# fuine/katome

Measured on AMD Instinct MI355X. Metric: k-mers/s, higher is better.
Workload: dtype u64

## Files before the change

### katome_amd/csrc/common.h

```cpp
#pragma once
#include <hip/hip_runtime.h>
#include <errno.h>
#include <stdarg.h>
#include <stdint.h>
#include <stdio.h>
#include <string.h>
#include <chrono>
#include <type_traits>
#include <vector>

#include "../../include/katome_gpu.h"
#include "env.h"
#include "kmer_bits.h"

namespace katome {

void set_error(const char* fmt, ...);
const char* get_error();

#define KCHECK_HIP(expr)                                                                         \
    do {                                                                                         \
        hipError_t _e = (expr);                                                                  \
        if (_e != hipSuccess) {                                                                  \
            katome::set_error("HIP error %d (%s) at %s:%d: %s", (int)_e, hipGetErrorString(_e),  \
// ... 144 lines not shown
    if (k < 3 || k > 63) { set_error("k = %u unsupported (3..63)", k); return KATOME_E_UNSUPPORTED; }
    return KATOME_OK;
}

constexpr int BLOCK = 256;
#ifdef __HIPCC__
__device__ __forceinline__ u32 wave_sum(u32 v) {
#pragma unroll
    for (int o = 32; o > 0; o >>= 1) v += __shfl_down(v, o, 64);
    return v;
}
#endif
inline unsigned grid_for(uint64_t work_items, unsigned per_block, unsigned cap = 256u * 16u) {
    uint64_t g = (work_items + per_block - 1) / per_block;
    if (g < 1) g = 1;
    return (unsigned)(g > cap ? cap : g);
}
#define KLAUNCH(kernel, n, stream, ...) hipLaunchKernelGGL(kernel, dim3(grid_for((n), BLOCK, 256u * 32u)), dim3(BLOCK), 0, stream, __VA_ARGS__)
inline double now_ms() { return std::chrono::duration<double, std::milli>(std::chrono::steady_clock::now().time_since_epoch()).count(); }

template <bool B> using BoolC = std::integral_constant<bool, B>;
template <int I> using IntC = std::integral_constant<int, I>;
template <class F> int with_bool(bool b, F f) { return b ? f(BoolC<true>{}) : f(BoolC<false>{}); }

int launch_extract_fixed(uint32_t k, bool rc, const uint8_t* d_packed, uint64_t n_reads, uint32_t read_len,
                         const uint8_t* d_skip, uint64_t* d_records, hipStream_t stream, uint32_t span = 1, bool mark = false,
                         uint32_t first_window = 0, uint32_t records_per_read = 0);
bool extract_tile_counts_ok(uint32_t k, uint32_t read_len, uint32_t span, uint32_t sort_tile, const uint8_t* d_packed, const uint64_t* d_records);
int launch_extract_tiles_counted(uint32_t k, bool rc, const uint8_t* d_packed, uint64_t n_reads, uint32_t read_len, uint32_t span,
                                 uint64_t* d_records, uint32_t* d_counts, uint32_t sort_tile, hipStream_t stream);
int launch_extract_var(uint32_t k, bool rc, const uint8_t* d_packed, uint64_t packed_bytes, const uint64_t* d_byte_off,
                       const uint32_t* d_len, const uint64_t* d_win_prefix, uint64_t n_reads, uint64_t total_windows,
                       uint64_t* d_records, hipStream_t stream, bool mark = false, uint32_t span = 1, uint32_t mode = 0);

int dev_sort(uint64_t* d_keys, uint32_t* d_vals, uint64_t n, uint32_t nw, uint32_t key_bits, hipStream_t stream);
struct DevBuf;
int dev_sort_bufs(DevBuf& keys, DevBuf* vals, uint64_t n, uint32_t nw, uint32_t key_bits, hipStream_t stream, bool distinct_keys = false);
int dev_partition(const uint64_t* d_in, const uint32_t* v_in, uint64_t n, uint32_t nw, uint32_t n_parts, uint64_t* d_out,
                  uint32_t* v_out, uint64_t* h_counts, hipStream_t stream, uint32_t core_shift = 0, uint32_t core_bases = 0, uint32_t minimizer = 0);
constexpr uint32_t SUPERMER_M = 11;
uint32_t supermer_slots(uint32_t k, uint32_t read_len, uint32_t m);
bool supermer_route_takes(uint32_t k, uint32_t read_len, uint32_t m);
int dev_supermers_extract(const uint8_t* d_packed, uint64_t n_reads, uint32_t read_len, const uint8_t* d_skip, uint32_t k, uint32_t m, bool rc,
                          uint32_t n_owners, uint32_t slots, uint64_t* d_out, uint64_t* d_spill, uint64_t spill_cap, uint64_t* d_spill_cursor,
                          hipStream_t stream);
int dev_supermers_expand(const uint64_t* d_list, const uint32_t* d_counts, uint64_t n, uint32_t k, bool rc, DevBuf& keys, DevBuf& weights,
                         uint64_t* n_records, hipStream_t stream);
int dev_partition_supermers(const uint64_t* d_in, uint64_t n, uint32_t n_parts, uint64_t* d_out, uint64_t* h_counts, hipStream_t stream);
int dev_partition_range(const uint64_t* d_vals, const uint32_t* idx_in, uint64_t n, const uint64_t* d_bounds, uint32_t n_parts,
                        uint64_t* d_out, uint32_t* idx_out, uint64_t* h_counts, hipStream_t stream);
int dev_hash_order_core(const uint64_t* d_in, const uint32_t* w_in, uint64_t n, uint32_t core_shift, uint32_t core_bases, uint64_t* ka, uint64_t* kb,
                        uint32_t* wa, uint32_t* wb, const uint64_t** k_out, const uint32_t** w_out, uint32_t* group_bits, hipStream_t stream);
inline bool fused_records_on() { static const bool on = env_flag("KATOME_FUSED_RECORDS", true); return on; }
struct RecordSource {
    const uint64_t* tiles = nullptr; const uint32_t* counts = nullptr;
    uint64_t n_tiles = 0;
    uint32_t tile_bases = 0, k = 0, span = 0, stride = 0;
    bool rc = false, rep = false, pending = false;
    DevBuf* keys = nullptr; DevBuf* weights = nullptr;
    size_t key_bytes = 0, weight_bytes = 0;
    hipStream_t stream = nullptr;
    DevBuf own_tiles, own_counts;
    uint64_t n_records() const { return n_tiles * span; }
    int first_pass_done() {
        pending = false; tiles = nullptr; counts = nullptr;
        own_tiles.release(); own_counts.release();
        if (int rc = keys->alloc(key_bytes, stream)) return rc;
        return weights->alloc(weight_bytes, stream);
    }
};
bool fused_records_takes(uint32_t nwt, uint32_t nwk, bool rep, uint32_t span);
int table_materialise_records(RecordSource& src);
int dev_hash_order_tagged(const uint64_t* d_in, const uint32_t* w_in, uint64_t n, uint32_t nwk, uint64_t* ka, uint64_t* kb, uint32_t* wa, uint32_t* wb,
                          const uint64_t** k_out, const uint32_t** w_out, uint32_t* group_bits, hipStream_t stream, uint32_t* first_counts = nullptr);
int dev_region_order(const uint64_t* d_in, const uint32_t* w_in, uint64_t n, uint32_t nw, int passes, uint64_t* ka, uint64_t* kb,
                     uint32_t* wa, uint32_t* wb, const uint64_t** k_out, const uint32_t** w_out, hipStream_t stream);
int dev_hash_order(const uint64_t* d_in, const uint32_t* w_in, uint64_t n, uint32_t nw, uint64_t* ka, uint64_t* kb, uint32_t* wa, uint32_t* wb,
                   const uint64_t** k_out, const uint32_t** w_out, uint32_t* group_bits, hipStream_t stream, uint32_t* first_counts = nullptr,
                   RecordSource* src = nullptr);
uint32_t dev_sort_tile_keys(uint32_t nw);
inline bool fused_hist_on() { static const bool on = env_flag("KATOME_FUSED_HIST", true); return on; }
int dev_key_order(const uint64_t* d_in, const uint32_t* w_in, uint64_t n, uint32_t k, uint64_t* ka, uint64_t* kb, uint32_t* wa, uint32_t* wb,
                  const uint64_t** k_out, const uint32_t** w_out, hipStream_t stream, uint32_t* first_counts = nullptr,
                  const uint8_t* first_digits = nullptr, RecordSource* src = nullptr);
int dev_list_first_pass(const uint64_t* d_tiles, const uint32_t* d_counts, uint64_t n_tiles, uint32_t tile_bases, uint32_t k, uint32_t span, uint32_t stride,
                        bool rc, bool rep, bool fused, uint64_t* d_keys, uint32_t* d_weights, uint32_t* d_digit_counts, hipStream_t stream);
int dev_s2_region_pass(const uint64_t* d_keys, const uint32_t* d_w, const uint8_t* d_digits, uint32_t k, const uint64_t* start, const uint64_t* used,
                       uint64_t* k_out, uint32_t* w_out, uint64_t* n_tiles, hipStream_t stream);
size_t dev_digit_stream_bytes(uint64_t n, uint32_t nw);
bool dev_digit_stream_pays(uint32_t nw);
int dev_key_group_index(const uint64_t* d_keys, uint64_t n, uint32_t shift, uint64_t* d_index, hipStream_t stream);
int dev_half_merge(const uint64_t* a_key, const uint32_t* a_w, const uint64_t* a_first, const uint32_t* a_count, const uint64_t* a_off,
                   const uint64_t* b_key, const uint32_t* b_w, const uint64_t* b_first, uint64_t* out_key, uint32_t* out_w, uint64_t n_out,
                   hipStream_t stream);
uint32_t dev_group_merge_cap();
uint64_t dev_source_head_blocks(uint64_t n_edges);
int dev_group_merge(const uint64_t* a_key, const uint32_t* a_w, const uint64_t* a_first, const uint32_t* a_count, const uint64_t* a_off,
                    const uint64_t* b_key, const uint32_t* b_w, const uint64_t* b_first, uint32_t k, uint64_t* out_key, uint32_t* out_w,
                    uint64_t n_out, hipStream_t stream, uint32_t* head_counts = nullptr);
int dev_key_group_max(const uint64_t* d_index, uint64_t* d_out, hipStream_t stream);
int dev_unique(uint64_t* d_keys, uint64_t n, uint32_t nw, uint64_t* n_out, hipStream_t stream);
int dev_rank(const uint64_t* d_sorted, uint64_t n_sorted, uint32_t nw, uint32_t key_bits, const uint64_t* d_q, uint64_t nq,
             uint64_t* d_out, hipStream_t stream);
int dev_bucket_index(const uint64_t* d_sorted, uint64_t n, uint32_t nw, uint32_t key_bits, uint32_t B, uint64_t* d_index, hipStream_t stream);
int dev_iota(uint32_t* d, uint64_t n, hipStream_t stream);
int dev_fill_u32(uint32_t* d, uint64_t n, uint32_t v, hipStream_t stream);
// ... 305 lines not shown
```

### katome_amd/csrc/radix.hip

```cpp
#include <algorithm>
#include <type_traits>

#include "common.h"
#include "edge_keys.h"
#include "lds_order.h"
#include "s2_regions.h"

namespace katome {

constexpr int RADIX_BITS = 8;
constexpr int RADIX = 1 << RADIX_BITS;
#ifndef KATOME_SORT_ITEMS
#define KATOME_SORT_ITEMS 16
#endif
#ifndef KATOME_SORT_ITEMS_WIDE
#define KATOME_SORT_ITEMS_WIDE 8
#endif
#ifndef KATOME_SORT_ITEMS_3
#define KATOME_SORT_ITEMS_3 5
#endif
#ifndef KATOME_SORT_WAVES
#define KATOME_SORT_WAVES 4
#endif
template <int NW> struct SortTile {
    static constexpr int ITEMS = NW == 1 ? KATOME_SORT_ITEMS : NW == 2 ? KATOME_SORT_ITEMS_WIDE : KATOME_SORT_ITEMS_3;
    static constexpr int KEYS = BLOCK * ITEMS;
};
static inline unsigned chunk_blocks_for(unsigned long long nblocks) {
    unsigned c = 64;
    while (c < 1024 && (unsigned long long)c * c < nblocks) c <<= 1;
    return c;
}
static_assert(BLOCK == RADIX, "one thread per digit in the offset kernels");

template <int NW> struct RadixDigit {
    u32 shift, bits;
    __device__ __forceinline__ u32 operator()(const Key<NW>& k) const { return key_digit(k, shift, bits); }
};
template <int NW> struct OwnerDigit {
    u64 n_parts;
    u32 core_shift, core_bases;
    u32 minimizer = 0;
    __device__ __forceinline__ u32 operator()(const Key<NW>& k0) const {
        if (!key_valid(k0)) return (u32)n_parts;
        Key<NW> k = k0;
        k.w[0] &= ~RC_MARK;
        if (minimizer) return (u32)minimizer_owner(k, core_shift, core_bases, minimizer, n_parts);
        return core_bases ? (u32)core_owner(k, core_shift, core_bases, n_parts) : (u32)whole_key_owner(k, n_parts);
    }
};
struct SupermerOwnerDigit {
    u32 n_parts;
    __device__ __forceinline__ u32 operator()(const Key<2>& k) const { return key_valid(k) ? supermer_owner(k) : n_parts; }
};
struct RangeDigit {
    const u64* bounds; u32 n_parts;
    __device__ __forceinline__ u32 operator()(const Key<1>& k) const {
// ... 112 lines not shown
    const u64 tile = nw == 1 ? SortTile<1>::KEYS : nw == 2 ? SortTile<2>::KEYS : SortTile<3>::KEYS;
    return (size_t)((n + tile - 1) / tile * tile);
}

__global__ __launch_bounds__(BLOCK) void radix_chunk_kernel(u32* __restrict__ counts, u64 nblocks, u64* __restrict__ chunk_sum, u32 chunk_blocks) {
    const u32 d = threadIdx.x;
    const u64 b0 = (u64)blockIdx.x * chunk_blocks;
    const u64 b1 = b0 + chunk_blocks < nblocks ? b0 + chunk_blocks : nblocks;
    u32 run = 0;
    constexpr int U = 8;
    u64 b = b0;
    for (; b + U <= b1; b += U) {
        u32 c[U];
#pragma unroll
        for (int j = 0; j < U; ++j) c[j] = counts[(b + j) * RADIX + d];
#pragma unroll
        for (int j = 0; j < U; ++j) { counts[(b + j) * RADIX + d] = run; run += c[j]; }
    }
    for (; b < b1; ++b) {
        u32 c = counts[b * RADIX + d];
        counts[b * RADIX + d] = run;
        run += c;
    }
    chunk_sum[(u64)blockIdx.x * RADIX + d] = run;
}

__global__ __launch_bounds__(BLOCK) void radix_offsets_kernel(u64* __restrict__ chunk_sum, u64 nchunks, u64* __restrict__ digit_total) {
    __shared__ u64 tot[RADIX];
    const u32 d = threadIdx.x;
    u64 t = 0;
    for (u64 c = 0; c < nchunks; ++c) t += chunk_sum[c * RADIX + d];
    tot[d] = t;
    if (digit_total) digit_total[d] = t;
    __syncthreads();
    u64 start = 0;
    for (u32 e = 0; e < d; ++e) start += tot[e];
    constexpr int U = 8;
    u64 c = 0;
    for (; c + U <= nchunks; c += U) {
        u64 v[U];
#pragma unroll
        for (int j = 0; j < U; ++j) v[j] = chunk_sum[(c + j) * RADIX + d];
#pragma unroll
        for (int j = 0; j < U; ++j) { chunk_sum[(c + j) * RADIX + d] = start; start += v[j]; }
    }
    for (; c < nchunks; ++c) {
        u64 v = chunk_sum[c * RADIX + d];
        chunk_sum[c * RADIX + d] = start;
        start += v;
    }
}

struct NoNextDigit {};
template <int NWT, int NWK, bool RC, bool REP> struct ListSource {
    static constexpr bool PLACED = false;
    const u64* tiles; const u32* counts; u32 k, span, stride, inv;
    struct Origin { u64 t0; u32 o0; };
    __device__ __forceinline__ Origin origin(u64 base) const { const u64 t0 = base / span; return Origin{t0, (u32)(base - t0 * span)}; }
    __device__ __forceinline__ void load(const Origin& at, u32 idx, Key<NWK>& key, u32& val) const {
        const u32 q = at.o0 + idx, tr = __umulhi(q, inv), o = q - tr * span;
        const u64 t = at.t0 + tr;
        Key<NWT> tile;
#pragma unroll
        for (int w = 0; w < NWT; ++w) tile.w[w] = tiles[t * NWT + w];
        key = level_orientation<NWK, RC, REP>(sub_window<NWT, NWK>(tile, k, span, stride, o), k);
        val = counts[t];
    }
};
template <class Next> struct NextDigitOut {
    Next nx; uint8_t* out;
    __device__ __forceinline__ void put(u64 at, u32 d) const { out[at] = (uint8_t)d; }
};
template <> struct NextDigitOut<NoNextDigit> {};
template <int NW, bool HAS_VAL, class Digit, bool STABLE = true, class Next = NoNextDigit, class Src = ArraySource>
__global__ __launch_bounds__(BLOCK, KATOME_SORT_WAVES) void radix_scatter_kernel(const u64* __restrict__ keys_in, const u32* __restrict__ vals_in,
                                                               u64 n, Digit dg, const u32* __restrict__ rel,
                                                               const u64* __restrict__ chunk_off, u64* __restrict__ keys_out,
                                                               u32* __restrict__ vals_out, u32 chunk_blocks, u32 xcd_tiles, NextDigitOut<Next> next, Src src) {
    constexpr bool NEXT = !std::is_same<Next, NoNextDigit>::value, PLACED = Src::PLACED, LISTED = !std::is_same<Src, ArraySource>::value && !PLACED;
    static_assert(!LISTED || HAS_VAL, "a list's records carry its counts");
    constexpr int SORT_ITEMS = SortTile<NW>::ITEMS, SORT_TILE = SortTile<NW>::KEYS;
    extern __shared__ u64 smem[];
    u64* skeys = smem;
    __shared__ u32 whist[BLOCK / 64][RADIX];
    __shared__ u32 dstart[RADIX];
    __shared__ u64 gbase[RADIX];
    __shared__ u32 wsum[BLOCK / 64];

    const u32 tid = threadIdx.x, lane = tid & 63, wave = tid >> 6;
    const u64 bid = xcd_tiles ? (u64)(blockIdx.x & 7u) * xcd_tiles + (blockIdx.x >> 3) : (u64)blockIdx.x;
    const u64 base = bid * SORT_TILE;
    if (base >= n) return;
    u32 cnt = (u32)((n - base) < (u64)SORT_TILE ? (n - base) : (u64)SORT_TILE);
    for (u32 i = tid; i < (BLOCK / 64) * RADIX; i += BLOCK) (&whist[0][0])[i] = 0;
    __syncthreads();

    Key<NW> key[SORT_ITEMS]; u32 val[SORT_ITEMS]; u32 dig[SORT_ITEMS]; u32 rnk[SORT_ITEMS];
    const u64 lt_mask = lane ? (~0ull >> (64 - lane)) : 0ull;
    const typename Src::Origin from = src.origin(base);
    u64 in0 = base;
    if constexpr (PLACED) { in0 = from.base; cnt = from.cnt; }
#pragma unroll
    for (int j = 0; j < SORT_ITEMS; ++j) {
        const u32 idx = wave * (64 * SORT_ITEMS) + j * 64 + lane;
        const bool valid = idx < cnt;
        u32 d = 0;
        if (valid) {
            if constexpr (LISTED) src.load(from, idx, key[j], val[j]);
            else {
#if KATOME_STREAM_LOADS >= 1
            key[j] = load_key_stream<NW>(keys_in, in0 + idx);
            if (HAS_VAL) val[j] = __builtin_nontemporal_load(&vals_in[in0 + idx]);
#else
            key[j] = load_key<NW>(keys_in, in0 + idx);
            if (HAS_VAL) val[j] = vals_in[in0 + idx];
#endif
            }
            d = dg(key[j]);
        }
        if (!STABLE) {
            dig[j] = d;
            rnk[j] = valid ? atomicAdd(&whist[0][d], 1u) : 0u;
            continue;
        }
        const u64 vmask = __ballot(valid);
        u32 diff_lo = 0, diff_hi = 0;
#pragma unroll
        for (int b = 0; b < RADIX_BITS; ++b) {
            const u32 mine = (u32)((int)(d << (31 - b)) >> 31);
            const u64 vote = __ballot(mine != 0);
            diff_lo |= (u32)vote ^ mine;
            diff_hi |= (u32)(vote >> 32) ^ mine;
        }
        const u64 m = ~((u64)diff_hi << 32 | diff_lo) & vmask;
        const u32 prior = __popcll(m & lt_mask);
        u32 old = 0;
        if (valid) old = whist[wave][d];
        if (valid && prior == 0) whist[wave][d] = old + __popcll(m);
        dig[j] = d;
        rnk[j] = old + prior;
    }
    __syncthreads();

    {
        const u32 d = tid;
        u32 run = 0;
        if (!STABLE) { run = whist[0][d]; whist[0][d] = 0; }
        else {
#pragma unroll
        for (int w = 0; w < BLOCK / 64; ++w) { u32 c = whist[w][d]; whist[w][d] = run; run += c; }
        }
        u32 incl = run;
#pragma unroll
        for (int o = 1; o < 64; o <<= 1) { u32 v = __shfl_up(incl, o, 64); if (lane >= (u32)o) incl += v; }
        if (lane == 63) wsum[wave] = incl;
        __syncthreads();
        u32 woff = 0;
#pragma unroll
        for (int w = 0; w < BLOCK / 64; ++w) if (w < (int)wave) woff += wsum[w];
        dstart[d] = woff + incl - run;
        gbase[d] = chunk_off[(bid / chunk_blocks) * RADIX + d] + rel[bid * RADIX + d];
    }
// ... 424 lines not shown
    PassBuffers pb;
    KCHECK(pb.init(n, (int)nw, stream));
    if (nw == 1) {
        OwnerDigit<1> dg{n_parts, core_shift, core_bases, minimizer};
        if (v_in) KCHECK((radix_pass<1, true>(d_in, v_in, n, dg, d_out, v_out, pb, stream)));
        else      KCHECK((radix_pass<1, false>(d_in, nullptr, n, dg, d_out, nullptr, pb, stream)));
    } else if (nw == 2) {
        OwnerDigit<2> dg{n_parts, core_shift, core_bases, minimizer};
        if (v_in) KCHECK((radix_pass<2, true>(d_in, v_in, n, dg, d_out, v_out, pb, stream)));
        else      KCHECK((radix_pass<2, false>(d_in, nullptr, n, dg, d_out, nullptr, pb, stream)));
    } else {
        OwnerDigit<3> dg{n_parts, core_shift, core_bases, minimizer};
        if (v_in) KCHECK((radix_pass<3, true>(d_in, v_in, n, dg, d_out, v_out, pb, stream)));
        else      KCHECK((radix_pass<3, false>(d_in, nullptr, n, dg, d_out, nullptr, pb, stream)));
    }
    u64 totals[RADIX];
    KCHECK_HIP(hipMemcpyAsync(totals, pb.totals.p, sizeof totals, hipMemcpyDeviceToHost, stream));
    KCHECK_HIP(hipStreamSynchronize(stream));
    for (u32 p = 0; p < n_parts; ++p) h_counts[p] = totals[p];
    return KATOME_OK;
}

int dev_partition_supermers(const uint64_t* d_in, uint64_t n, uint32_t n_parts, uint64_t* d_out, uint64_t* h_counts, hipStream_t stream) {
    if (n_parts == 0 || n_parts > 16) { set_error("supermers: 1..16 owners"); return KATOME_E_ARG; }
    for (u32 p = 0; p < n_parts; ++p) h_counts[p] = 0;
    if (n == 0) return KATOME_OK;
    PassBuffers pb;
    KCHECK(pb.init(n, 2, stream));
    SupermerOwnerDigit dg{n_parts};
    KCHECK((radix_pass<2, false>(d_in, nullptr, n, dg, d_out, nullptr, pb, stream)));
    u64 totals[RADIX];
    KCHECK_HIP(hipMemcpyAsync(totals, pb.totals.p, sizeof totals, hipMemcpyDeviceToHost, stream));
    KCHECK_HIP(hipStreamSynchronize(stream));
    for (u32 p = 0; p < n_parts; ++p) h_counts[p] = totals[p];
    return KATOME_OK;
}

int dev_partition_range(const uint64_t* d_vals, const uint32_t* idx_in, uint64_t n, const uint64_t* d_bounds, uint32_t n_parts,
                        uint64_t* d_out, uint32_t* idx_out, uint64_t* h_counts, hipStream_t stream) {
    if (n_parts == 0 || n_parts >= (u32)RADIX) { set_error("n_parts must be 1..255"); return KATOME_E_ARG; }
    for (u32 p = 0; p < n_parts; ++p) h_counts[p] = 0;
    if (n == 0) return KATOME_OK;
    PassBuffers pb;
    KCHECK(pb.init(n, 1, stream));
    RangeDigit dg{d_bounds, n_parts};
    KCHECK((radix_pass<1, true>(d_vals, idx_in, n, dg, d_out, idx_out, pb, stream)));
    u64 totals[RADIX];
    KCHECK_HIP(hipMemcpyAsync(totals, pb.totals.p, sizeof totals, hipMemcpyDeviceToHost, stream));
    KCHECK_HIP(hipStreamSynchronize(stream));
    for (u32 p = 0; p < n_parts; ++p) h_counts[p] = totals[p];
    return KATOME_OK;
}

template <int NWT, int NWK, bool RC, bool REP> static ListSource<NWT, NWK, RC, REP> list_source(const RecordSource& s) {
    return ListSource<NWT, NWK, RC, REP>{s.tiles, s.counts, s.k, s.span, s.stride, (u32)((1ull << 32) / s.span) + 1};
}
static bool source_by_key(const RecordSource& s) {
    return s.rep && key_words_for_k(s.k) == 1 && fused_records_takes((u32)key_words_for_k(s.tile_bases), 1, true, s.span);
}
static bool source_by_hash(const RecordSource& s, u32 nw) {
    return !s.rep && nw == 2 && (u32)key_words_for_k(s.k) == 2 && fused_records_takes((u32)key_words_for_k(s.tile_bases), 2, false, s.span);
}
static int list_pass_by_key(const RecordSource& s, u64 n, u32 k, u64* ka, u32* wa, PassBuffers& pb, hipStream_t stream) {
    const LevelKeyDigit dg{2 * k - 16};
    return with_bool(s.rc, [&](auto rcv) {
        constexpr bool RC = decltype(rcv)::value;
        if (key_words_for_k(s.tile_bases) == 2)
            return radix_pass<1, true, LevelKeyDigit, true, NoNextDigit>(nullptr, nullptr, n, dg, ka, wa, pb, stream, true, nullptr, NoNextDigit{}, nullptr, list_source<2, 1, RC, true>(s));
        return radix_pass<1, true, LevelKeyDigit, true, NoNextDigit>(nullptr, nullptr, n, dg, ka, wa, pb, stream, true, nullptr, NoNextDigit{}, nullptr, list_source<1, 1, RC, true>(s));
    });
}
static int list_pass_by_hash(const RecordSource& s, u64 n, u64* ka, u32* wa, PassBuffers& pb, uint8_t* digits, hipStream_t stream) {
    const HashDigit<2> dg{48u}, nx{56u};
    return with_bool(s.rc, [&](auto rcv) {
        return radix_pass<2, true, HashDigit<2>, true, HashDigit<2>>(nullptr, nullptr, n, dg, ka, wa, pb, stream, true, nullptr, nx, digits, list_source<2, 2, decltype(rcv)::value, false>(s));
    });
}

template <int NW>
static int region_order_t(const u64* d_in, const u32* w_in, u64 n, int passes, u64* ka, u64* kb, u32* wa, u32* wb,
                          const u64** k_out, const u32** w_out, hipStream_t stream, u32* first_counts = nullptr, RecordSource* src = nullptr) {
    PassBuffers pb;
    KCHECK(pb.init(n, NW, stream));
    const bool listed = src && src->pending && passes == 2 && first_counts && digit_stream_pays(NW) && !unstable_first() && source_by_hash(*src, NW);
    if (src && src->pending && !listed) {
        KCHECK(table_materialise_records(*src));
        d_in = kb = src->keys->as<u64>(); w_in = wb = src->weights->as<u32>();
    }
    pb.first = first_counts;
    DevBuf digits(stream);
    const u64* kin = d_in; const u32* win = w_in;
    u64* kdst[2] = {ka, kb}; u32* wdst[2] = {wa, wb};
    const bool has_w = w_in || listed;
    for (int p = 0; p < passes; ++p) {
        HashDigit<NW> dg{(u32)(64 - 8 * (passes - p))};
        const bool have = p == 0 && first_counts != nullptr;
        if (order_trace() && passes == 2 && p == 0)
            fprintf(stderr, "[order] by hash: %llu records of %d words, first pass counted from %s, second from %s\n", (unsigned long long)n, NW,
                    have ? "its writer's counts" : "the keys", digit_stream_pays(NW) && !unstable_first() ? "the digit stream" : "the keys");
        if constexpr (digit_stream_pays(NW)) if (passes == 2 && !unstable_first()) {
            if (p == 0) {
                KCHECK(digits.alloc(digit_stream_bytes(n, NW)));
                const HashDigit<NW> nx{56u};
                if (listed) {
                    if constexpr (NW == 2) KCHECK(list_pass_by_hash(*src, n, kdst[0], wdst[0], pb, digits.as<uint8_t>(), stream));
                    KCHECK(src->first_pass_done());
                    kdst[1] = src->keys->as<u64>(); wdst[1] = src->weights->as<u32>();
                    kin = kdst[0]; win = wdst[0];
                    continue;
                }
                if (w_in) KCHECK((radix_pass<NW, true, HashDigit<NW>, true, HashDigit<NW>>(kin, win, n, dg, kdst[0], wdst[0], pb, stream, have, nullptr, nx, digits.as<uint8_t>())));
                else      KCHECK((radix_pass<NW, false, HashDigit<NW>, true, HashDigit<NW>>(kin, nullptr, n, dg, kdst[0], nullptr, pb, stream, have, nullptr, nx, digits.as<uint8_t>())));
            } else {
                if (has_w) KCHECK((radix_pass<NW, true>(kin, win, n, dg, kdst[1], wdst[1], pb, stream, false, digits.as<uint8_t>())));
                else      KCHECK((radix_pass<NW, false>(kin, nullptr, n, dg, kdst[1], nullptr, pb, stream, false, digits.as<uint8_t>())));
            }
            kin = kdst[p & 1]; win = has_w ? wdst[p & 1] : nullptr;
            continue;
        }
        if (p == 0 && unstable_first()) {
            if (w_in) KCHECK((radix_pass<NW, true, HashDigit<NW>, false>(kin, win, n, dg, kdst[p & 1], wdst[p & 1], pb, stream, have)));
            else      KCHECK((radix_pass<NW, false, HashDigit<NW>, false>(kin, nullptr, n, dg, kdst[p & 1], nullptr, pb, stream, have)));
        } else
        if (w_in) KCHECK((radix_pass<NW, true>(kin, win, n, dg, kdst[p & 1], wdst[p & 1], pb, stream, have)));
        else      KCHECK((radix_pass<NW, false>(kin, nullptr, n, dg, kdst[p & 1], nullptr, pb, stream, have)));
        kin = kdst[p & 1]; win = w_in ? wdst[p & 1] : nullptr;
    }
    *k_out = kin; *w_out = win;
    return KATOME_OK;
// ... 605 lines not shown
```

### katome_amd/csrc/table.hip

```cpp
#include <atomic>
#include <cstdio>
#include <vector>

#include "common.h"
#include "lds_plan.h"
#include "seq_pair.h"
#include "slot_bits.h"

namespace katome {

struct Slot1 { u64 key; u32 count; u32 pad; };
struct Slot2 { u64 hi; u64 lo; u32 count; u32 pad[3]; };
struct Slot3 { u64 hi; u64 mid; u64 lo; u32 count; u32 pad; };
static_assert(sizeof(Slot1) == 16 && sizeof(Slot2) == 32 && sizeof(Slot3) == 32, "slot layout");

__device__ __forceinline__ u64 ld_agent(const u64* p) { return __hip_atomic_load(p, __ATOMIC_RELAXED, __HIP_MEMORY_SCOPE_AGENT); }
__device__ __forceinline__ void st_agent(u64* p, u64 v) { __hip_atomic_store(p, v, __ATOMIC_RELAXED, __HIP_MEMORY_SCOPE_AGENT); }

__device__ __forceinline__ u32 upsert(Slot1* slots, u64 cap, Key<1> key, u32 add, u32* err, u64* slot_out = nullptr) {
    const u64 want = key.w[0] | OCC;
    u64 s = hash_to_range(hash_key(key), cap);
    for (u64 probes = 0; probes < cap; ++probes) {
        u64 cur = slots[s].key;
        u32 fresh = 0;
        if (cur == 0) {
            cur = atomicCAS(&slots[s].key, 0ull, want);
            if (cur == 0) { cur = want; fresh = 1; }
        }
        if (cur == want) {
            atomicAdd(&slots[s].count, add);
            if (slot_out) *slot_out = s;
            return fresh;
        }
        if (++s == cap) s = 0;
    }
    *err = 1;
    return 0;
}

struct SeenInit { u64* seen; u64 a, b; bool both; };
__device__ __forceinline__ void seen_store(const SeenInit& si, u64 s) {
    st_agent(&si.seen[2 * s], si.a);
    if (si.both) st_agent(&si.seen[2 * s + 1], si.b);
}
__device__ __forceinline__ u32 upsert(Slot2* slots, u64 cap, Key<2> key, u32 add, u32* err, u64* slot_out = nullptr, const SeenInit* si = nullptr) {
    u64 s = hash_to_range(hash_key(key), cap);
    u64 spins = 0;
    for (u64 probes = 0; probes < cap;) {
        u64 cur = slots[s].hi;
        bool cached_view = true;
        if (cur != 0 && !(cur & OCC)) { cur = ld_agent(&slots[s].hi); cached_view = false; }
        asm volatile("" ::: "memory");
        if (cur == 0) {
            cur = atomicCAS(&slots[s].hi, 0ull, key.w[0] | LOCK);
            cached_view = false;
            if (cur == 0) {
                st_agent(&slots[s].lo, key.w[1]);
// ... 441 lines not shown
            for (int q = 0; q < NWK; ++q) out_keys[(base + p) * NWK + q] = x.w[q];
            out_w[base + p] = lcnt[t];
        }
        __syncthreads();
    }
}

template <int NWT, int NWK, bool RC, bool REP = false>
__global__ __launch_bounds__(BLOCK) void list_to_records_kernel(const u64* __restrict__ tiles, const u32* __restrict__ counts, u64 n_tiles, u32 k, u32 span,
                                                                 u32 stride, u64* __restrict__ out_keys, u32* __restrict__ out_w) {
    const u64 n = n_tiles * span;
    for (u64 p = (u64)blockIdx.x * BLOCK + threadIdx.x; p < n; p += (u64)gridDim.x * BLOCK) {
        const u64 t = p / span;
        const u32 o = (u32)(p - t * span);
        Key<NWT> tile;
#pragma unroll
        for (int q = 0; q < NWT; ++q) tile.w[q] = tiles[t * NWT + q];
        const Key<NWK> x = level_orientation<NWK, RC, REP>(sub_window<NWT, NWK>(tile, k, span, stride, o), k);
#pragma unroll
        for (int q = 0; q < NWK; ++q) out_keys[p * NWK + q] = x.w[q];
        out_w[p] = counts[t];
    }
}

template <int NWT, int NWK, bool RC, bool REP = false>
__global__ __launch_bounds__(BLOCK) void list_to_records_hist_kernel(const u64* __restrict__ tiles, const u32* __restrict__ counts, u64 n_tiles, u32 k, u32 span,
                                                                      u32 stride, u64* __restrict__ out_keys, u32* __restrict__ out_w, u32 tile_keys,
                                                                      u32* __restrict__ digit_counts) {
    static_assert(BLOCK == 256, "one thread per digit");
    __shared__ u32 h[256];
    const u64 n = n_tiles * span, n_out_tiles = (n + tile_keys - 1) / tile_keys;
    for (u64 ot = blockIdx.x; ot < n_out_tiles; ot += gridDim.x) {
        h[threadIdx.x] = 0;
        __syncthreads();
        const u64 p0 = ot * tile_keys, p1 = p0 + tile_keys < n ? p0 + tile_keys : n;
        for (u64 p = p0 + threadIdx.x; p < p1; p += BLOCK) {
            const u64 t = p / span;
            const u32 o = (u32)(p - t * span);
            Key<NWT> tile;
#pragma unroll
            for (int q = 0; q < NWT; ++q) tile.w[q] = tiles[t * NWT + q];
            const Key<NWK> x = level_orientation<NWK, RC, REP>(sub_window<NWT, NWK>(tile, k, span, stride, o), k);
#pragma unroll
            for (int q = 0; q < NWK; ++q) out_keys[p * NWK + q] = x.w[q];
            out_w[p] = counts[t];
            atomicAdd(&h[(REP ? (u32)(x.w[0] >> (2 * k - 16)) : (u32)(hash_key(x) >> 48)) & 255u], 1u);
        }
        __syncthreads();
        digit_counts[ot * 256 + threadIdx.x] = h[threadIdx.x];
        __syncthreads();
    }
}

template <int NWT, int NWK, bool RC, bool REP = false>
__global__ __launch_bounds__(BLOCK) void list_digit_counts_kernel(const u64* __restrict__ tiles, u64 n_tiles, u32 k, u32 span, u32 stride, u32 inv, u32 tile_keys,
                                                                   u32* __restrict__ digit_counts) {
    static_assert(BLOCK == 256, "one thread per digit");
    __shared__ u32 h[256];
    const u64 n = n_tiles * span, n_out_tiles = (n + tile_keys - 1) / tile_keys;
    for (u64 ot = blockIdx.x; ot < n_out_tiles; ot += gridDim.x) {
        h[threadIdx.x] = 0;
        __syncthreads();
        const u64 p0 = ot * tile_keys, t0 = p0 / span;
        const u32 o0 = (u32)(p0 - t0 * span), cnt = (u32)(n - p0 < (u64)tile_keys ? n - p0 : (u64)tile_keys);
        for (u32 i = threadIdx.x; i < cnt; i += BLOCK) {
            const u32 q = o0 + i, tr = __umulhi(q, inv), o = q - tr * span;
            const u64 t = t0 + tr;
            Key<NWT> tile;
#pragma unroll
            for (int w = 0; w < NWT; ++w) tile.w[w] = tiles[t * NWT + w];
            const Key<NWK> x = sub_window<NWT, NWK>(tile, k, span, stride, o);
            u32 d;
            if constexpr (REP) {
                const u32 own = (u32)(x.w[0] >> (2 * k - 16)) & 255u;
                u32 v = ~(u32)(x.w[0] >> 8) & 255u;
                v = ((v & 0x0Fu) << 4) | (v >> 4);
                v = ((v & 0x33u) << 2) | ((v >> 2) & 0x33u);
                d = RC && ((x.w[0] >> k) & 1ull) ? v : own;
            } else d = (u32)(hash_key(level_orientation<NWK, RC, false>(x, k)) >> 48) & 255u;
            atomicAdd(&h[d], 1u);
        }
        __syncthreads();
        digit_counts[ot * 256 + threadIdx.x] = h[threadIdx.x];
        __syncthreads();
    }
}


constexpr int KR_ITEMS = 8;
template <int NW, bool TAGGED>
__global__ __launch_bounds__(BLOCK) void keep_rest_kernel(const u64* __restrict__ rec, u64 n, u64 read0, u32 per_read, u32 win0, u32 seq_per_read,
                                                           u64* __restrict__ out, unsigned long long* cursor, u32 win_stride, u32 span) {
    constexpr int WORDS = NW + (TAGGED ? 1 : 0);
    constexpr u32 TILE = BLOCK * KR_ITEMS;
    __shared__ u32 wtot[KR_ITEMS][BLOCK / 64];
    __shared__ unsigned long long base_sh;
    const u32 tid = threadIdx.x, lane = tid & 63, wave = tid >> 6;
    const u64 lt_mask = lane ? (~0ull >> (64 - lane)) : 0ull;
    for (u64 t0 = (u64)blockIdx.x * TILE; t0 < n; t0 += (u64)gridDim.x * TILE) {
        Key<NW> key[KR_ITEMS];
        u32 before[KR_ITEMS];
#pragma unroll
        for (int j = 0; j < KR_ITEMS; ++j) {
            const u64 i = t0 + (u64)j * BLOCK + tid;
            key[j] = key_invalid<NW>();
            if (i < n) {
#pragma unroll
                for (int q = 0; q < NW; ++q) key[j].w[q] = rec[i * NW + q];
            }
            const u64 m = __ballot(key_valid(key[j]));
            before[j] = __popcll(m & lt_mask);
            if (lane == 0) wtot[j][wave] = __popcll(m);
        }
        __syncthreads();
        if (tid == 0) {
            u32 run = 0;
#pragma unroll
// ... 414 lines not shown
                                  uint32_t stride, bool rc, bool rep, u64* d_keys, u32* d_weights, hipStream_t stream) {
    const dim3 grid(grid_for(n_tiles * span, BLOCK, 256u * 32u)), block(BLOCK);
    KernelScope ks(K_RECORDS, stream, n_tiles);
#define KATOME_LR(NWT, NWK, REP) with_bool(rc, [&](auto rcv) { hipLaunchKernelGGL((list_to_records_kernel<NWT, NWK, decltype(rcv)::value, REP>), grid, block, 0, stream, d_tiles, d_counts, n_tiles, k, span, stride, d_keys, d_weights); return 0; })
    if (rep) { if (nwt == 2) KATOME_LR(2, 1, true); else KATOME_LR(1, 1, true); }
    else if (nwt == 3 && nwk == 3) KATOME_LR(3, 3, false);
    else if (nwt == 3 && nwk == 2) KATOME_LR(3, 2, false);
    else if (nwt == 2 && nwk == 2) KATOME_LR(2, 2, false);
    else if (nwt == 2 && nwk == 1) KATOME_LR(2, 1, false);
    else if (nwt == 1 && nwk == 1) KATOME_LR(1, 1, false);
    else { set_error("records of a tile list: tiles of %u words into windows of %u", nwt, nwk); return KATOME_E_UNSUPPORTED; }
#undef KATOME_LR
    KCHECK_HIP(hipGetLastError());
    return KATOME_OK;
}

bool fused_records_takes(uint32_t nwt, uint32_t nwk, bool rep, uint32_t span) {
    if (span < 2 || span > 64) return false;
    return rep ? (nwk == 1 && nwt <= 2) : (nwt == 2 && nwk == 2);
}

int table_materialise_records(RecordSource& s) {
    if (!s.pending) return KATOME_OK;
    KCHECK(s.keys->alloc(s.key_bytes, s.stream));
    KCHECK(s.weights->alloc(s.weight_bytes, s.stream));
    if (getenv("KATOME_LC_TRACE")) fprintf(stderr, "[records] %llu records written after all: wanted before their first pass\n", (unsigned long long)s.n_records());
    KCHECK(launch_list_to_records(s.tiles, s.counts, s.n_tiles, (uint32_t)key_words_for_k(s.tile_bases), (uint32_t)key_words_for_k(s.k), s.k, s.span, s.stride,
                                  s.rc, s.rep, s.keys->as<u64>(), s.weights->as<u32>(), s.stream));
    s.pending = false; s.tiles = nullptr; s.counts = nullptr;
    s.own_tiles.release(); s.own_counts.release();
    return KATOME_OK;
}

int table_list_to_records(const uint64_t* d_tiles, const uint32_t* d_counts, uint64_t n_tiles, uint32_t tile_bases, uint32_t k, uint32_t span, uint32_t stride, bool rc,
                          DevBuf& keys, DevBuf& weights, uint64_t* n_records, hipStream_t stream, uint64_t extra_room, DevBuf* first_counts, bool rep,
                          RecordSource* src) {
    const uint32_t nwt = (uint32_t)key_words_for_k(tile_bases), nwk = (uint32_t)key_words_for_k(k);
    if (rep && (nwk != 1 || nwt > 2 || k < 9 || (rc && !(k & 1)))) { set_error("records in their representative orientation: one-word k-mers, k >= 9, odd k or one strand"); return KATOME_E_ARG; }
    *n_records = n_tiles * span;
    const bool counted = first_counts && fused_hist_on() && !extra_room && ((nwt == 3 && nwk >= 2) || (nwt == 2 && nwk <= 2) || (nwt == 1 && nwk == 1));
    const bool fused = src && counted && *n_records && fused_records_on() && fused_records_takes(nwt, nwk, rep, span);
    if (src && getenv("KATOME_LC_TRACE"))
        fprintf(stderr, "[records] %llu records of %u words off a list of %llu: %s\n", (unsigned long long)*n_records, nwk, (unsigned long long)n_tiles,
                fused ? "made by their first partition pass" : !fused_records_on() ? "written (KATOME_FUSED_RECORDS=0)"
                : extra_room ? "written (left-over windows go behind them)" : !counted ? "written (no counts for the first pass)"
                : !*n_records ? "written (none)" : "written (this shape's first pass reads records)");
    const uint32_t tile_keys = dev_sort_tile_keys(nwk);
    const uint64_t n_out_tiles = (*n_records + tile_keys - 1) / tile_keys;
    const dim3 hgrid(grid_for(n_out_tiles, 1, 256u * 32u)), block(BLOCK);
    if (fused) {
        keys.release(); weights.release();
        KCHECK(first_counts->alloc(n_out_tiles * 256 * 4 + 16, stream));
        const uint32_t inv = (uint32_t)((1ull << 32) / span) + 1;
        KernelScope ks(K_RECORDS, stream, n_tiles);
#define KATOME_LDC(NWT, NWK, REP) with_bool(rc, [&](auto rcv) { hipLaunchKernelGGL((list_digit_counts_kernel<NWT, NWK, decltype(rcv)::value, REP>), hgrid, block, 0, stream, d_tiles, n_tiles, k, span, stride, inv, tile_keys, first_counts->as<u32>()); return 0; })
        if (rep) { if (nwt == 2) KATOME_LDC(2, 1, true); else KATOME_LDC(1, 1, true); }
        else KATOME_LDC(2, 2, false);
#undef KATOME_LDC
        KCHECK_HIP(hipGetLastError());
        src->tiles = d_tiles; src->counts = d_counts; src->n_tiles = n_tiles;
        src->tile_bases = tile_bases; src->k = k; src->span = span; src->stride = stride; src->rc = rc; src->rep = rep;
        src->keys = &keys; src->weights = &weights; src->key_bytes = (*n_records + 1) * 8 * nwk; src->weight_bytes = (*n_records + 1) * 4;
        src->stream = stream; src->pending = true;
        return KATOME_OK;
    }
    KCHECK(keys.alloc((*n_records + extra_room + 1) * 8 * nwk, stream));
    KCHECK(weights.alloc((*n_records + extra_room + 1) * 4, stream));
    if (*n_records == 0) return KATOME_OK;
    if (counted) {
        KCHECK(first_counts->alloc(n_out_tiles * 256 * 4 + 16, stream));
        KernelScope ks(K_RECORDS, stream, n_tiles);
#define KATOME_LRH(NWT, NWK, REP) with_bool(rc, [&](auto rcv) { hipLaunchKernelGGL((list_to_records_hist_kernel<NWT, NWK, decltype(rcv)::value, REP>), hgrid, block, 0, stream, d_tiles, d_counts, n_tiles, k, span, stride, keys.as<u64>(), weights.as<u32>(), tile_keys, first_counts->as<u32>()); return 0; })
        if (rep) { if (nwt == 2) KATOME_LRH(2, 1, true); else KATOME_LRH(1, 1, true); }
        else if (nwt == 3 && nwk == 3) KATOME_LRH(3, 3, false);
        else if (nwt == 3 && nwk == 2) KATOME_LRH(3, 2, false);
        else if (nwt == 2 && nwk == 2) KATOME_LRH(2, 2, false);
        else if (nwt == 2 && nwk == 1) KATOME_LRH(2, 1, false);
        else KATOME_LRH(1, 1, false);
#undef KATOME_LRH
        KCHECK_HIP(hipGetLastError());
        return KATOME_OK;
    }
    if (first_counts) first_counts->release();
    return launch_list_to_records(d_tiles, d_counts, n_tiles, nwt, nwk, k, span, stride, rc, rep, keys.as<u64>(), weights.as<u32>(), stream);
}

int table_tiles_to_records_fast(Table& tiles, uint32_t k, uint32_t span, bool rc, DevBuf& keys, DevBuf& weights, uint64_t* n_records, hipStream_t stream,
                                uint64_t extra_room) {
    uint64_t occ = 0;
    KCHECK(table_occupied(tiles, &occ, stream));
    const uint32_t nwk = (uint32_t)key_words_for_k(k);
    const bool streaming = (nwk == 1 && (tiles.nw == 1 || tiles.nw == 2)) || (nwk == 2 && (tiles.nw == 2 || tiles.nw == 3));
    if (!streaming) {
        if (extra_room) { set_error("records of this tile shape cannot be extended"); return KATOME_E_UNSUPPORTED; }
        return table_expand_tiles_to_records(tiles, k, span, rc, keys, weights, n_records, stream, nullptr);
    }
    KCHECK(keys.alloc((occ * span + extra_room + 1) * 8 * nwk, stream));
    KCHECK(weights.alloc((occ * span + extra_room + 1) * 4, stream));
    DevBuf cursor(stream);
    KCHECK(cursor.alloc(8));
    KCHECK_HIP(hipMemsetAsync(cursor.p, 0, 8, stream));
    dim3 grid(grid_for(tiles.cap, BLOCK * TR_ITEMS, 256u * 8u)), block(BLOCK);
    KernelScope ks(K_RECORDS, stream, tiles.cap);
#define KATOME_TR(NWT, NWK) with_bool(rc, [&](auto rcv) { hipLaunchKernelGGL((tiles_to_records_kernel<NWT, NWK, decltype(rcv)::value>), grid, block, 0, stream, tiles.slots.as<SlotOf<NWT>::type>(), tiles.cap, k, span, 1u, keys.as<u64>(), weights.as<u32>(), cursor.as<u64>()); return 0; })
    if (nwk == 1) { if (tiles.nw == 1) KATOME_TR(1, 1); else KATOME_TR(2, 1); }
    else          { if (tiles.nw == 2) KATOME_TR(2, 2); else KATOME_TR(3, 2); }
#undef KATOME_TR
    KCHECK_HIP(hipGetLastError());
// ... 169 lines not shown
```

Baseline: 180.7 billion.

## Decode list entries once per entry and stage records in LDS

In the fused-records path, each thread now loads one list entry (tile) and cuts all of its span windows, instead of every record reloading its tile and recomputing the window with a reverse complement. The scatter kernel stages the resulting keys in shared memory before the per-item loop, and the digit-count kernel likewise iterates per entry. This is meant to cut redundant global tile loads and repeated revcomp work. In exchange it adds an extra LDS pass and a sync, and work per thread becomes uneven when the tile count is not a multiple of span. It is gated by KATOME_ENTRY_CUT, which is on by default.

```diff
diff --git a/katome_amd/csrc/common.h b/katome_amd/csrc/common.h
--- a/katome_amd/csrc/common.h
+++ b/katome_amd/csrc/common.h
@@ -220,6 +220,7 @@
 int dev_hash_order_core(const uint64_t* d_in, const uint32_t* w_in, uint64_t n, uint32_t core_shift, uint32_t core_bases, uint64_t* ka, uint64_t* kb,
                         uint32_t* wa, uint32_t* wb, const uint64_t** k_out, const uint32_t** w_out, uint32_t* group_bits, hipStream_t stream);
 inline bool fused_records_on() { static const bool on = env_flag("KATOME_FUSED_RECORDS", true); return on; }
+inline bool entry_cut_on() { static const bool on = env_flag("KATOME_ENTRY_CUT", true); return on; }
 struct RecordSource {
     const uint64_t* tiles = nullptr; const uint32_t* counts = nullptr;
     uint64_t n_tiles = 0;
diff --git a/katome_amd/csrc/entry_cut.h b/katome_amd/csrc/entry_cut.h
--- /dev/null
+++ b/katome_amd/csrc/entry_cut.h
@@ -0,0 +1,24 @@
+#pragma once
+#include "kmer_bits.h"
+
+namespace katome {
+
+template <int NWT, int NWK, bool RC, bool REP> struct EntryCut {
+    static_assert(!REP || NWK == 1, "the representative orientation is one of one-word k-mers");
+    Key<NWT> fwd, rev;
+    u32 bits, step, top;
+    KD EntryCut(const Key<NWT>& tile, u32 sub_len, u32 span, u32 stride) : fwd(tile), rev(tile), bits(2 * sub_len), step(2 * stride), top(2 * stride * (span - 1)) {
+        if (RC) rev = revcomp(tile, sub_len + stride * (span - 1));
+    }
+    KD Key<NWK> forward(u32 o) const { return narrow_key(key_low_bits(key_shr(fwd, top - step * o), bits), (Key<NWK>*)nullptr); }
+    KD Key<NWK> reverse(u32 o) const { return narrow_key(key_low_bits(key_shr(rev, step * o), bits), (Key<NWK>*)nullptr); }
+    KD Key<NWK> record(u32 o) const {
+        const Key<NWK> f = forward(o);
+        if (!RC) return f;
+        const Key<NWK> r = reverse(o);
+        if (REP) return ((f.w[0] >> (bits >> 1)) & 1ull) ? r : f;
+        return key_lt(r, f) ? r : f;
+    }
+};
+
+}
diff --git a/katome_amd/csrc/radix.hip b/katome_amd/csrc/radix.hip
--- a/katome_amd/csrc/radix.hip
+++ b/katome_amd/csrc/radix.hip
@@ -3,6 +3,7 @@
 
 #include "common.h"
 #include "edge_keys.h"
+#include "entry_cut.h"
 #include "lds_order.h"
 #include "s2_regions.h"
 
@@ -221,8 +222,8 @@
 }
 
 struct NoNextDigit {};
-template <int NWT, int NWK, bool RC, bool REP> struct ListSource {
-    static constexpr bool PLACED = false;
+template <int NWT, int NWK, bool RC, bool REP, bool ENTRY_CUT = true> struct ListSource {
+    static constexpr bool PLACED = false, ENTRY = ENTRY_CUT;
     const u64* tiles; const u32* counts; u32 k, span, stride, inv;
     struct Origin { u64 t0; u32 o0; };
     __device__ __forceinline__ Origin origin(u64 base) const { const u64 t0 = base / span; return Origin{t0, (u32)(base - t0 * span)}; }
@@ -235,6 +236,25 @@
         key = level_orientation<NWK, RC, REP>(sub_window<NWT, NWK>(tile, k, span, stride, o), k);
         val = counts[t];
     }
+    __device__ __forceinline__ void stage(const Origin& at, u32 cnt, u64* skeys, u32 tid) const {
+        const u32 n_ent = (at.o0 + cnt + span - 1) / span;
+        for (u32 e = tid; e < n_ent; e += BLOCK) {
+            Key<NWT> tile;
+#pragma unroll
+            for (int w = 0; w < NWT; ++w) tile.w[w] = tiles[(at.t0 + e) * NWT + w];
+            const EntryCut<NWT, NWK, RC, REP> cut(tile, k, span, stride);
+            const u32 first = e * span - at.o0;
+            for (u32 o = 0; o < span; ++o) {
+                const u32 idx = first + o;
+                if (idx < cnt) {
+                    const Key<NWK> x = cut.record(o);
+#pragma unroll
+                    for (int w = 0; w < NWK; ++w) skeys[idx * NWK + w] = x.w[w];
+                }
+            }
+        }
+    }
+    __device__ __forceinline__ u32 count_of(const Origin& at, u32 idx) const { return counts[at.t0 + __umulhi(at.o0 + idx, inv)]; }
 };
 template <class Next> struct NextDigitOut {
     Next nx; uint8_t* out;
@@ -262,6 +282,7 @@
     if (base >= n) return;
     u32 cnt = (u32)((n - base) < (u64)SORT_TILE ? (n - base) : (u64)SORT_TILE);
     for (u32 i = tid; i < (BLOCK / 64) * RADIX; i += BLOCK) (&whist[0][0])[i] = 0;
+    if constexpr (LISTED) if constexpr (Src::ENTRY) src.stage(src.origin(base), cnt, skeys, tid);
     __syncthreads();
 
     Key<NW> key[SORT_ITEMS]; u32 val[SORT_ITEMS]; u32 dig[SORT_ITEMS]; u32 rnk[SORT_ITEMS];
@@ -275,8 +296,13 @@
         const bool valid = idx < cnt;
         u32 d = 0;
         if (valid) {
-            if constexpr (LISTED) src.load(from, idx, key[j], val[j]);
-            else {
+            if constexpr (LISTED) {
+                if constexpr (Src::ENTRY) {
+#pragma unroll
+                    for (int q = 0; q < NW; ++q) key[j].w[q] = skeys[idx * NW + q];
+                    val[j] = src.count_of(from, idx);
+                } else src.load(from, idx, key[j], val[j]);
+            } else {
 #if KATOME_STREAM_LOADS >= 1
             key[j] = load_key_stream<NW>(keys_in, in0 + idx);
             if (HAS_VAL) val[j] = __builtin_nontemporal_load(&vals_in[in0 + idx]);
@@ -807,8 +833,8 @@
     return KATOME_OK;
 }
 
-template <int NWT, int NWK, bool RC, bool REP> static ListSource<NWT, NWK, RC, REP> list_source(const RecordSource& s) {
-    return ListSource<NWT, NWK, RC, REP>{s.tiles, s.counts, s.k, s.span, s.stride, (u32)((1ull << 32) / s.span) + 1};
+template <int NWT, int NWK, bool RC, bool REP, bool ENTRY> static ListSource<NWT, NWK, RC, REP, ENTRY> list_source(const RecordSource& s) {
+    return ListSource<NWT, NWK, RC, REP, ENTRY>{s.tiles, s.counts, s.k, s.span, s.stride, (u32)((1ull << 32) / s.span) + 1};
 }
 static bool source_by_key(const RecordSource& s) {
     return s.rep && key_words_for_k(s.k) == 1 && fused_records_takes((u32)key_words_for_k(s.tile_bases), 1, true, s.span);
@@ -818,18 +844,19 @@
 }
 static int list_pass_by_key(const RecordSource& s, u64 n, u32 k, u64* ka, u32* wa, PassBuffers& pb, hipStream_t stream) {
     const LevelKeyDigit dg{2 * k - 16};
-    return with_bool(s.rc, [&](auto rcv) {
-        constexpr bool RC = decltype(rcv)::value;
+    return with_bool(s.rc, [&](auto rcv) { return with_bool(entry_cut_on(), [&](auto cutv) {
+        constexpr bool RC = decltype(rcv)::value, CUT = decltype(cutv)::value;
         if (key_words_for_k(s.tile_bases) == 2)
-            return radix_pass<1, true, LevelKeyDigit, true, NoNextDigit>(nullptr, nullptr, n, dg, ka, wa, pb, stream, true, nullptr, NoNextDigit{}, nullptr, list_source<2, 1, RC, true>(s));
-        return radix_pass<1, true, LevelKeyDigit, true, NoNextDigit>(nullptr, nullptr, n, dg, ka, wa, pb, stream, true, nullptr, NoNextDigit{}, nullptr, list_source<1, 1, RC, true>(s));
-    });
+            return radix_pass<1, true, LevelKeyDigit, true, NoNextDigit>(nullptr, nullptr, n, dg, ka, wa, pb, stream, true, nullptr, NoNextDigit{}, nullptr, list_source<2, 1, RC, true, CUT>(s));
+        return radix_pass<1, true, LevelKeyDigit, true, NoNextDigit>(nullptr, nullptr, n, dg, ka, wa, pb, stream, true, nullptr, NoNextDigit{}, nullptr, list_source<1, 1, RC, true, CUT>(s));
+    }); });
 }
 static int list_pass_by_hash(const RecordSource& s, u64 n, u64* ka, u32* wa, PassBuffers& pb, uint8_t* digits, hipStream_t stream) {
     const HashDigit<2> dg{48u}, nx{56u};
-    return with_bool(s.rc, [&](auto rcv) {
-        return radix_pass<2, true, HashDigit<2>, true, HashDigit<2>>(nullptr, nullptr, n, dg, ka, wa, pb, stream, true, nullptr, nx, digits, list_source<2, 2, decltype(rcv)::value, false>(s));
-    });
+    return with_bool(s.rc, [&](auto rcv) { return with_bool(entry_cut_on(), [&](auto cutv) {
+        return radix_pass<2, true, HashDigit<2>, true, HashDigit<2>>(nullptr, nullptr, n, dg, ka, wa, pb, stream, true, nullptr, nx, digits,
+                                                                      list_source<2, 2, decltype(rcv)::value, false, decltype(cutv)::value>(s));
+    }); });
 }
 
 template <int NW>
diff --git a/katome_amd/csrc/table.hip b/katome_amd/csrc/table.hip
--- a/katome_amd/csrc/table.hip
+++ b/katome_amd/csrc/table.hip
@@ -3,6 +3,7 @@
 #include <vector>
 
 #include "common.h"
+#include "entry_cut.h"
 #include "lds_plan.h"
 #include "seq_pair.h"
 #include "slot_bits.h"
@@ -550,7 +551,7 @@
     }
 }
 
-template <int NWT, int NWK, bool RC, bool REP = false>
+template <int NWT, int NWK, bool RC, bool REP = false, bool ENTRY = true>
 __global__ __launch_bounds__(BLOCK) void list_digit_counts_kernel(const u64* __restrict__ tiles, u64 n_tiles, u32 k, u32 span, u32 stride, u32 inv, u32 tile_keys,
                                                                    u32* __restrict__ digit_counts) {
     static_assert(BLOCK == 256, "one thread per digit");
@@ -561,6 +562,30 @@
         __syncthreads();
         const u64 p0 = ot * tile_keys, t0 = p0 / span;
         const u32 o0 = (u32)(p0 - t0 * span), cnt = (u32)(n - p0 < (u64)tile_keys ? n - p0 : (u64)tile_keys);
+        if constexpr (ENTRY) {
+            const u32 n_ent = (o0 + cnt + span - 1) / span;
+            for (u32 e = threadIdx.x; e < n_ent; e += BLOCK) {
+                Key<NWT> tile;
+#pragma unroll
+                for (int w = 0; w < NWT; ++w) tile.w[w] = tiles[(t0 + e) * NWT + w];
+                const u32 first = e * span - o0;
+                if constexpr (REP) {
+                    for (u32 o = 0; o < span; ++o) {
+                        const u32 s = 2 * stride * (span - 1 - o);
+                        const u32 own = key_digit(tile, s + 2 * k - 16, 8);
+                        u32 v = ~key_digit(tile, s + 8, 8) & 255u;
+                        v = ((v & 0x0Fu) << 4) | (v >> 4);
+                        v = ((v & 0x33u) << 2) | ((v >> 2) & 0x33u);
+                        const u32 d = RC && key_digit(tile, s + k, 1) ? v : own;
+                        if (first + o < cnt) atomicAdd(&h[d], 1u);
+                    }
+                } else {
+                    const EntryCut<NWT, NWK, RC, false> cut(tile, k, span, stride);
+                    for (u32 o = 0; o < span; ++o)
+                        if (first + o < cnt) atomicAdd(&h[(u32)(hash_key(cut.record(o)) >> 48) & 255u], 1u);
+                }
+            }
+        } else
         for (u32 i = threadIdx.x; i < cnt; i += BLOCK) {
             const u32 q = o0 + i, tr = __umulhi(q, inv), o = q - tr * span;
             const u64 t = t0 + tr;
@@ -1081,8 +1106,9 @@
         keys.release(); weights.release();
         KCHECK(first_counts->alloc(n_out_tiles * 256 * 4 + 16, stream));
         const uint32_t inv = (uint32_t)((1ull << 32) / span) + 1;
+        if (getenv("KATOME_LC_TRACE")) fprintf(stderr, "[entry_cut] %s\n", entry_cut_on() ? "once per list entry" : "once per record (KATOME_ENTRY_CUT=0)");
         KernelScope ks(K_RECORDS, stream, n_tiles);
-#define KATOME_LDC(NWT, NWK, REP) with_bool(rc, [&](auto rcv) { hipLaunchKernelGGL((list_digit_counts_kernel<NWT, NWK, decltype(rcv)::value, REP>), hgrid, block, 0, stream, d_tiles, n_tiles, k, span, stride, inv, tile_keys, first_counts->as<u32>()); return 0; })
+#define KATOME_LDC(NWT, NWK, REP) with_bool(rc, [&](auto rcv) { return with_bool(entry_cut_on(), [&](auto cutv) { hipLaunchKernelGGL((list_digit_counts_kernel<NWT, NWK, decltype(rcv)::value, REP, decltype(cutv)::value>), hgrid, block, 0, stream, d_tiles, n_tiles, k, span, stride, inv, tile_keys, first_counts->as<u32>()); return 0; }); })
         if (rep) { if (nwt == 2) KATOME_LDC(2, 1, true); else KATOME_LDC(1, 1, true); }
         else KATOME_LDC(2, 2, false);
 #undef KATOME_LDC
```

New measurement: 183.4 billion, median of 6. 1.02x the previous value.
